# databio/IGD

Hardware: AMD Instinct MI355X
Metric: query-intervals/sec (igd search -q, hits-only) on roadmap-scale synthetic .igd (higher is better)
Workload: dtype int32; 1 GPU; BASELINE config 2: roadmap-scale synthetic IGD, 1900 files x 26316 intervals (53143736 tile records, 188505 tiles of 16384 bp, hg38 contigs) replicated per GPU + 1000000 position-sorted queries per step (seed 7), hits-only, queries and DB resident in HBM; queries_per_gpu=1000000, parallelism=query-sharded x1, grouping=sorted, query_layout=contig numbers + starts + ends (12 B/query; igd_hip_search_dev), collective=none

## Files before the change

### igd_amd/csrc/engine/host_search.hpp

```cpp

static int ensure_workspace(igd_hip_db *db, int64_t nq, int pairBytes)
{
    int rc;
    if (nq > db->wsQueries) {
        HIPCHK(hipDeviceSynchronize());
        if (db->d_fix) (void)hipFree(db->d_fix);
        if (db->d_qw) (void)hipFree(db->d_qw);
        if (db->d_later) (void)hipFree(db->d_later);
        if (db->d_laterHdr) (void)hipFree(db->d_laterHdr);
        db->d_fix = nullptr; db->d_qw = nullptr; db->d_later = nullptr; db->d_laterHdr = nullptr;
        db->wsQueries = 0;
        if ((rc = dalloc(&db->d_fix, (size_t)nq * 2, nullptr)) != IGD_HIP_OK) return rc;
        if ((rc = dalloc(&db->d_qw, (size_t)nq + 64, nullptr)) != IGD_HIP_OK) return rc;
        if ((rc = dalloc(&db->d_later, (size_t)nq + 4096 + 64, nullptr)) != IGD_HIP_OK) return rc;
        if ((rc = dalloc(&db->d_laterHdr, 2 * ((size_t)nq / 256 + 2), nullptr)) != IGD_HIP_OK) return rc;
        db->wsQueries = nq;
    }
    if (pairBytes == 0 || (nq <= db->wsBucket && pairBytes <= db->pairBytes)) return IGD_HIP_OK;
    HIPCHK(hipDeviceSynchronize());
    const int64_t cap = nq > db->wsBucket ? nq : db->wsBucket;
    const int pb = pairBytes > db->pairBytes ? pairBytes : db->pairBytes;
    {
        void *ws[] = { db->d_pairs, db->d_long, db->d_spTable, db->d_spT, db->d_spSub };
        for (void *q : ws) if (q) (void)hipFree(q);
        db->d_pairs = nullptr; db->d_long = nullptr; db->d_spTable = nullptr; db->d_spT = nullptr; db->d_spSub = nullptr;
    }
    db->wsBucket = 0;
    if ((rc = dalloc((char **)&db->d_pairs, (size_t)cap * IGD_SHORT_TILES * (size_t)pb, nullptr)) != IGD_HIP_OK) return rc;
    if ((rc = dalloc(&db->d_long, (size_t)cap, nullptr)) != IGD_HIP_OK) return rc;
    {
        int sh = SP_MINSHIFT;
        while (sh < 13 && ((db->nT + (1 << sh) - 1) >> sh) > SP_MAXC) sh++;
        db->spShift = (((db->nT + (1 << sh) - 1) >> sh) <= SP_MAXC && sh <= 12) ? sh : -1;
        db->spCoarse = db->spShift >= 0 ? (db->nT + (1 << sh) - 1) >> sh : 0;
        if (db->spShift >= 0) {
            const size_t nWG = (size_t)((cap + SP_Q - 1) / SP_Q);
            if ((rc = dalloc(&db->d_spTable, nWG * (size_t)db->spCoarse, nullptr)) != IGD_HIP_OK) return rc;
            if ((rc = dalloc(&db->d_spT, nWG * SP_CAP, nullptr)) != IGD_HIP_OK) return rc;
            const size_t subN = (((size_t)db->spCoarse * SPF_S) << db->spShift) + 2 * (size_t)db->spCoarse + 16;
            if ((rc = dalloc(&db->d_spSub, subN, nullptr)) != IGD_HIP_OK) return rc;
            HIPCHK(hipMemset(db->d_spSub, 0, subN * 4));
        }
    }
    db->wsBucket = cap;
    db->pairBytes = pb;
    return IGD_HIP_OK;
}

static int launch_bucket(igd_hip_db *db, const int32_t *d_ichr, const int32_t *d_qs, const int32_t *d_qe,
                         int nq, int rule, int gate, int packed, hipStream_t st, u64 *zeroHits = nullptr,
                         u64 *zeroTotal = nullptr)
{
    const int nT = db->nT;
    const int qb = (nq + 255) / 256;
    const int qbz = zeroHits ? ((nq > db->nFiles ? nq : db->nFiles) + 255) / 256 : qb;
    k_count_pairs<<<qbz, 256, 0, st>>>(db->v, d_ichr, d_qs, d_qe, nq, rule, packed, db->d_pairCnt, db->d_long, db->d_ctl,
                                      gate, db->epoch, zeroHits, zeroTotal);
    const int sb = (nT + IGD_SCAN_TILE - 1) / IGD_SCAN_TILE;
    k_scan_block_sums<<<sb, IGD_SCAN_BLOCK, 0, st>>>(db->d_pairCnt, nT, db->d_blockSums, db->d_ctl, gate);
    k_scan_apply<<<sb, IGD_SCAN_BLOCK, 0, st>>>(db->d_pairCnt, nT, db->d_blockSums, db->d_pairPos, db->d_pairN,
                                                db->d_ctl, gate);
    k_scatter_pairs<<<qb, 256, 0, st>>>(db->v, d_ichr, d_qs, d_qe, nq, rule, packed, db->d_pairPos, db->d_pairs,
                                                db->d_ctl, gate);
    HIPCHK(hipGetLastError());
    return IGD_HIP_OK;
}

static int launch_split(igd_hip_db *db, const int32_t *d_ichr, const int32_t *d_qs, const int32_t *d_qe,
                        int nq, int rule, int gate, int packed, hipStream_t st, u64 *zeroHits, u64 *zeroTotal)
{
    const int nWG = (nq + SP_Q - 1) / SP_Q;
    uint32_t *bases = db->d_spSub + (((size_t)db->spCoarse * SPF_S) << db->spShift);
    int32_t *blong = (int32_t *)(bases + db->spCoarse);
    const int bitsWords = (!db->splitNoBits && db->v.tileBits && db->nT <= 40 * 1024 * 8) ? (db->nT + 31) / 32 + 1 : 0;
    const int ctgStaged = (!db->splitNoBits && db->nCtg <= 1024) ? db->nCtg : 0;
    const int stageCap = (db->splitNoBits || db->splitNoRegion) ? 0 : SP_Q + SP_Q / 8;
    size_t ldsLocal = (size_t)bitsWords * 4 + (size_t)ctgStaged * 8;
    if (ldsLocal < (size_t)stageCap * 12 + 16) ldsLocal = (size_t)stageCap * 12 + 16;
    if (bitsWords && ctgStaged && db->v.vshift < 0 && db->v.shift >= 0 && db->spShift >= 2)
    k_split_local<true><<<nWG, SP_WG, ldsLocal, st>>>(db->v, d_ichr, d_qs, d_qe, nq, rule, packed, db->spShift, db->spCoarse, db->d_spTable,
                                         db->d_spT, db->d_long, db->d_ctl, gate, db->epoch, zeroHits, zeroTotal, blong, bitsWords, ctgStaged, stageCap);
    else
    k_split_local<false><<<nWG, SP_WG, ldsLocal, st>>>(db->v, d_ichr, d_qs, d_qe, nq, rule, packed, db->spShift, db->spCoarse, db->d_spTable,
                                         db->d_spT, db->d_long, db->d_ctl, gate, db->epoch, zeroHits, zeroTotal, blong, bitsWords, ctgStaged, stageCap);
    const size_t ldsCnt = (size_t)2 * 4 << db->spShift;
    int64_t cap = 2 * (((int64_t)nq + nq / 8) / db->spCoarse) + 256;
    if (cap < 1024) cap = 1024;
    if (cap > (int64_t)((65536 - 256 - ldsCnt) / 12)) cap = (int64_t)((65536 - 256 - ldsCnt) / 12);
    if (db->splitNoStage || cap < 256) cap = 0;
    k_split_fine_a<<<db->spCoarse * SPF_S, SPF_WG, ldsCnt + (size_t)cap * 12, st>>>(db->nT, db->spShift, db->spCoarse, nWG, db->d_spTable, db->d_spT,
        db->d_spSub, bases, blong, db->d_pairN, db->d_pairPos, (int2 *)db->d_pairs, db->d_ctl, gate, db->d_ctl, db->epoch, packed ? db->d_heavy : nullptr, (int)cap);
    k_split_fine_b<<<db->spCoarse * SPF_S < 512 ? db->spCoarse * SPF_S : 512, SPF_WG, (size_t)4 << db->spShift, st>>>(db->nT, db->spShift, db->spCoarse, nWG, db->d_spTable, db->d_spT,
        db->d_spSub, bases, blong, db->d_pairN, db->d_pairPos, (int2 *)db->d_pairs, db->d_ctl, gate, db->d_ctl, db->epoch, packed ? db->d_heavy : nullptr);
    HIPCHK(hipGetLastError());
    return IGD_HIP_OK;
}

static SortK make_sortk(igd_hip_db *db, const ScanArgs &a)
{
    SortArgs sa;
    sa.firstQ = a.firstQ; sa.spill = db->d_spill; sa.qw0 = db->d_qw; sa.later = db->d_later; sa.q_qs = a.q_qs; sa.ctl = a.ctl;
    sa.laterHdr = (const int2 *)db->d_laterHdr; sa.lbShift = db->lbShift; sa.lpos = db->d_lpos;
    sa.nq = a.nq; sa.v = a.v; sa.epoch = a.epoch; sa.mode = a.mode; sa.out = a.out; sa.rule = a.rule;
    sa.sbCap = db->sbCap; sa.wldsBytes = IGD_WLDS_BYTES + 2 * db->sbCap;
    sa.ctlw = db->d_ctl; sa.heavyS = db->d_heavy + IGD_HEAVY_MAX; sa.farList = db->d_far; sa.tailHistOff = -1; sa.noList = 0;
    SortK K;
    K.db = db->v; K.a = sa; K.hitsOut = (u64 *)a.hitsOut; K.totalOut = a.total;
    return K;
}

template <typename F, typename KA>
static void launch_sorted(igd_hip_db *db, F kernel, int grid, int block, size_t lds, hipStream_t st, const KA &K)
{
    if (db->evStart) {
        KA k = K;
        void *args[] = {&k};
        (void)hipExtLaunchKernel((const void *)kernel, dim3(grid), dim3(block), args, lds, st, db->evStart, db->evStop, 0);
        db->evStart = db->evStop = nullptr;
    } else kernel<<<grid, block, lds, st>>>(K);
}

template <bool USE_V, bool LDS_HITS, bool PACKED>
static void launch_scan(igd_hip_db *db, const ScanArgs &a, hipStream_t st, int win = -1)
{
    const int fileLo = win > 0 ? win * db->winN : 0;
    const int fileN = win >= 0 ? (db->nFiles - fileLo < db->winN ? db->nFiles - fileLo : db->winN) : db->nFiles;
    const size_t lds = LDS_HITS ? db->ldsBytes : 0;
    if (a.mode != 2 && PACKED) {
        const bool big = db->bigImage || db->nRec + IGD_CHUNK >= (1ll << 30);
        const size_t ldsS = (size_t)db->ldsSorted;
        SortK K = make_sortk(db, a);
        if (win >= 0) { K.db.nFiles = fileN; K.db.fileLo = fileLo; K.hitsOut += fileLo; K.a.noList = win > 0 ? 1 : 0; }
        const int forceRank = db->forceRank;
        bool lean = forceRank >= 0 ? forceRank == 0 : ((int64_t)a.nq < 28ll * db->nT && (int64_t)a.nq >= (int64_t)db->nT);
        const int64_t wavesLean = (int64_t)db->grid * (IGD_WG_LEAN / IGD_WAVE);
        if (((int64_t)db->nUnits + wavesLean - 1) / wavesLean * (IGD_WG_LEAN / IGD_WAVE) * (IGD_LEAN_FIRST + IGD_WAVE) * IGD_CHUNK >= (1ll << 32)) lean = false;
        const int few = (LDS_HITS && !big) ? (win >= 0 ? 3 : db->nFiles == 1 ? 1 : db->nFiles <= 8 ? 2 : 0) : 0;
        if (big) launch_sorted(db, igd_scan_sorted<USE_V, LDS_HITS, LDS_HITS, true, true>, db->grid, IGD_WG_RANK, ldsS, st, K);
        else if (lean) {
            const size_t l = LDS_HITS ? ldsS : 0;
            if (few == 1) launch_sorted(db, igd_scan_sorted<USE_V, LDS_HITS, LDS_HITS, false, false, LDS_HITS ? 1 : 0>, db->grid, IGD_WG_LEAN, l, st, K);
            else if (few == 2) launch_sorted(db, igd_scan_sorted<USE_V, LDS_HITS, LDS_HITS, false, false, LDS_HITS ? 2 : 0>, db->grid, IGD_WG_LEAN, l, st, K);
            else if (few == 3) launch_sorted(db, igd_scan_sorted<USE_V, LDS_HITS, LDS_HITS, false, false, LDS_HITS ? 3 : 0>, db->grid, IGD_WG_LEAN, l, st, K);
            else launch_sorted(db, igd_scan_sorted<USE_V, LDS_HITS, LDS_HITS, false, false>, db->grid, IGD_WG_LEAN, l, st, K);
        } else {
            if (few == 1) launch_sorted(db, igd_scan_sorted<USE_V, LDS_HITS, LDS_HITS, false, true, LDS_HITS ? 1 : 0>, db->grid, IGD_WG_RANK, ldsS, st, K);
            else if (few == 2) launch_sorted(db, igd_scan_sorted<USE_V, LDS_HITS, LDS_HITS, false, true, LDS_HITS ? 2 : 0>, db->grid, IGD_WG_RANK, ldsS, st, K);
            else if (few == 3) launch_sorted(db, igd_scan_sorted<USE_V, LDS_HITS, LDS_HITS, false, true, LDS_HITS ? 3 : 0>, db->grid, IGD_WG_RANK, ldsS, st, K);
            else launch_sorted(db, igd_scan_sorted<USE_V, LDS_HITS, LDS_HITS, false, true>, db->grid, IGD_WG_RANK, ldsS, st, K);
        }
    } else
    if (a.mode != 2) {
        if (win >= 0) { DbView v = db->v; v.nFiles = fileN; v.fileLo = fileLo; igd_scan_tiles<true, USE_V, LDS_HITS, PACKED, LDS_HITS><<<db->grid, IGD_WG, lds, st>>>(v, a); }
        else igd_scan_tiles<true, USE_V, LDS_HITS, PACKED><<<db->grid, IGD_WG, lds, st>>>(db->v, a);
    }
    if (a.mode != 1) {
        if (win >= 0) { DbView v = db->v; v.nFiles = fileN; v.fileLo = fileLo; igd_scan_tiles<false, USE_V, LDS_HITS, PACKED, LDS_HITS><<<db->grid, IGD_WG, lds, st>>>(v, a); }
        else igd_scan_tiles<false, USE_V, LDS_HITS, PACKED><<<db->grid, IGD_WG, lds, st>>>(db->v, a);
    }
}
template <bool LDS_HITS>
static void launch_scan_any(igd_hip_db *db, const ScanArgs &a, bool useV, bool packed, hipStream_t st, int win = -1)
{
    if (packed) {
        if (useV) launch_scan<true, LDS_HITS, true>(db, a, st, win); else launch_scan<false, LDS_HITS, true>(db, a, st, win);
    } else {
        if (useV) launch_scan<true, LDS_HITS, false>(db, a, st, win); else launch_scan<false, LDS_HITS, false>(db, a, st, win);
    }
}

__global__ void k_expand_runs(const int32_t *__restrict__ runs, int nCtg, int32_t *__restrict__ ichr, int nq)
{
    const int i = blockIdx.x * blockDim.x + threadIdx.x;
    if (i >= nq) return;
    int lo = 0, hi = nCtg;
    while (hi - lo > 1) { const int mid = (lo + hi) >> 1; if (runs[mid] <= i) lo = mid; else hi = mid; }
    ichr[i] = lo;
}

static int search_dev_impl(igd_hip_db *db, const int32_t *d_ichr, const int32_t *d_runs, const int32_t *d_qs,
                           const int32_t *d_qe, int64_t nq, int32_t v, int rule, int flags,
                           int64_t *d_hits, int64_t *d_total, void *stream);

extern "C" int igd_hip_search_dev(igd_hip_db *db, const int32_t *d_ichr, const int32_t *d_qs,
                                  const int32_t *d_qe, int64_t nq, int32_t v, int rule, int flags,
                                  int64_t *d_hits, int64_t *d_total, void *stream)
{
    return search_dev_impl(db, d_ichr, nullptr, d_qs, d_qe, nq, v, rule, flags, d_hits, d_total, stream);
}

extern "C" int igd_hip_search_runs_dev(igd_hip_db *db, const int32_t *d_run_start, const int32_t *d_qs,
                                       const int32_t *d_qe, int64_t nq, int32_t v, int rule, int flags,
                                       int64_t *d_hits, int64_t *d_total, void *stream)
{
    if (!d_run_start || (flags & IGD_HIP_FLAG_BUCKET)) {
        snprintf(g_err, sizeof g_err, "igd_hip_search_runs_dev: bad argument");
        return IGD_HIP_ERR_ARG;
    }
    return search_dev_impl(db, nullptr, d_run_start, d_qs, d_qe, nq, v, rule, flags | IGD_HIP_FLAG_SORTED, d_hits, d_total, stream);
}

static int search_dev_impl(igd_hip_db *db, const int32_t *d_ichr, const int32_t *d_runs, const int32_t *d_qs,
                           const int32_t *d_qe, int64_t nq, int32_t v, int rule, int flags,
                           int64_t *d_hits, int64_t *d_total, void *stream)
{
    if (!db || !d_hits || nq < 0 || nq > IGD_MAX_BATCH || (rule != IGD_HIP_RULE_NEST && rule != IGD_HIP_RULE_FLAT) ||
        ((flags & IGD_HIP_FLAG_SORTED) && (flags & IGD_HIP_FLAG_BUCKET))) {
        snprintf(g_err, sizeof g_err, "igd_hip_search_dev: bad argument");
        return IGD_HIP_ERR_ARG;
    }
    if (db->nFiles == 0) return IGD_HIP_OK;
    if (db->inner) {
        db->inner->vnest = rule == IGD_HIP_RULE_NEST ? 1 : 0;
        return search_dev_impl(db->inner, d_ichr, d_runs, d_qs, d_qe, nq, v, IGD_HIP_RULE_FLAT, flags, d_hits, d_total,
                               stream ? stream : (void *)db->stream);
    }
    HIPCHK(hipSetDevice(db->device));
    hipStream_t st = stream ? (hipStream_t)stream : db->stream;
    if (nq == 0 || db->nT == 0) {
        if (flags & IGD_HIP_FLAG_ZERO_FIRST) {
            HIPCHK(hipMemsetAsync(d_hits, 0, (size_t)db->nFiles * 8, st));
            if (d_total) HIPCHK(hipMemsetAsync(d_total, 0, 8, st));
        }
        return IGD_HIP_OK;
    }
    int rc = ensure_workspace(db, nq, (flags & IGD_HIP_FLAG_SORTED) ? 0 : 8);
    if (rc != IGD_HIP_OK) return rc;
    const bool useV = (v != IGD_HIP_NO_VALUE_FILTER && db->gType == 1);
    const int mode = (flags & IGD_HIP_FLAG_SORTED) ? 1 : (flags & IGD_HIP_FLAG_BUCKET) ? 2 : 0;
    const int krule = rule | ((db->v.vshift >= 0 && db->vnest) ? 0x100 : 0);
    const bool packed = db->packed && !(flags & IGD_HIP_FLAG_EXACT) && (!useV || db->packedV);
    if (db->epoch >= 0x3fffffff || db->covStale) {
        HIPCHK(hipMemsetAsync(db->d_spill, 0, ((size_t)db->nT + 2) * 4, st));
        HIPCHK(hipMemsetAsync(db->d_cov, 0, 4 * IGD_COV_LEN(db->nT) * 4, st));
        HIPCHK(hipMemsetAsync(db->d_ctl + CTL_COV, 0, 4 * 4, st));
        if (db->d_spSub && db->spShift >= 0)
            HIPCHK(hipMemsetAsync(db->d_spSub + (((size_t)db->spCoarse * SPF_S) << db->spShift) + db->spCoarse, 0, (size_t)db->spCoarse * 4, st));
        if (!db->covStale) db->epoch = 0;
        db->covStale = false;
    }
    db->epoch++;
    struct StaleGuard { igd_hip_db *d; bool done; ~StaleGuard() { if (!done) d->covStale = true; } } guard{db, false};
    int slot = -1;
    if (db->evOn && db->evUsed < db->evMax && (db->evSeen++ % (db->evEvery > 0 ? db->evEvery : 1)) == 0) slot = db->evUsed++;
    const bool pipeEv = slot >= 0 && slot < IGD_PIPE_EVENTS;
    if (pipeEv) HIPCHK(hipEventRecord(db->ev[4 * slot + 0], st));
    u64 *zh = (flags & IGD_HIP_FLAG_ZERO_FIRST) ? (u64 *)d_hits : nullptr;
    u64 *zt = (flags & IGD_HIP_FLAG_ZERO_FIRST) ? (u64 *)d_total : nullptr;
    const bool direct = mode == 1 && packed && db->ldsHits && db->nWin == 1 && db->v.tileD != nullptr && db->v.vshift < 0 && db->v.shift >= 0 && db->nCtg <= QB_CTG &&
                        (db->forceDirect > 0 || (db->forceDirect < 0 && (flags & IGD_HIP_FLAG_SHORT) && nq >= 28ll * db->nT));
    db->lastDirect = direct ? 1 : 0;
    if (mode != 2) {
        bool vec = ((((uintptr_t)d_ichr) | ((uintptr_t)d_qs) | ((uintptr_t)d_qe)) & 15) == 0;
        const bool fast = packed && db->v.shift >= 0 && db->nCtg <= QB_CTG;
        if (nq < 65536) vec = false;
        bool runsK = d_runs != nullptr && vec && fast;
        if (d_runs && !runsK) {
            if (nq > db->runCap) {
                HIPCHK(hipStreamSynchronize(st));
                if (db->d_runIchr) (void)hipFree(db->d_runIchr);
                db->d_runIchr = nullptr; db->runCap = 0;
                if ((rc = dalloc(&db->d_runIchr, (size_t)nq, nullptr)) != IGD_HIP_OK) return rc;
                db->runCap = nq;
            }
            k_expand_runs<<<(int)((nq + 255) / 256), 256, 0, st>>>(d_runs, db->nCtg, db->d_runIchr, (int)nq);
            d_ichr = db->d_runIchr;
            vec = vec && (((uintptr_t)d_ichr) & 15) == 0;
        }
        const int fillBlocks = (int)((db->nT >> 10) < 256 ? (db->nT >> 10) + 1 : 256);
        const bool wide = vec && nq >= ((int64_t)1 << 22);
#define QB_GRID(PER_) ((int)((nq + (PER_) - 1) / (PER_)) > fillBlocks ? (int)((nq + (PER_) - 1) / (PER_)) : fillBlocks)
#define QB_LAUNCH(VEC_, FAST_, WGT_)                                                                                                  \
    if (direct && FAST_ && runsK && VEC_ == 4)                                         \
        k_query_bounds<4, true, WGT_, true, true><<<QB_GRID(WGT_ * 4), WGT_, 0, st>>>(db->v, d_runs, d_qs, d_qe, (int)nq, krule,      \
        1, db->d_firstQ, db->d_lpos, db->d_fix, db->d_ctl, db->epoch, zh, zt, db->d_qw, db->d_later, db->d_spill,                      \
        (int2 *)db->d_laterHdr, 1);                                                                                                  \
    else if (direct && FAST_)                                                                                                        \
        k_query_bounds<VEC_, true, WGT_, false, true><<<QB_GRID(WGT_ * VEC_), WGT_, 0, st>>>(db->v, d_ichr, d_qs, d_qe, (int)nq, krule, \
        1, db->d_firstQ, db->d_lpos, db->d_fix, db->d_ctl, db->epoch, zh, zt, db->d_qw, db->d_later, db->d_spill,                      \
        (int2 *)db->d_laterHdr, 1);                                                                                                  \
    else if (runsK && VEC_ == 4 && FAST_)                                                                                             \
        k_query_bounds<4, true, WGT_, true><<<QB_GRID(WGT_ * 4), WGT_, 0, st>>>(db->v, d_runs, d_qs, d_qe, (int)nq, krule,            \
        packed ? 1 : 0, db->d_firstQ, db->d_lpos, db->d_fix, db->d_ctl, db->epoch, zh, zt, db->d_qw, db->d_later, db->d_spill,         \
        (int2 *)db->d_laterHdr, mode == 1 ? 1 : 0);                                                                                  \
    else                                                                                                                             \
    k_query_bounds<VEC_, FAST_, WGT_><<<QB_GRID(WGT_ * VEC_), WGT_, 0, st>>>(db->v, d_ichr, d_qs, d_qe, (int)nq, krule,               \
        packed ? 1 : 0, db->d_firstQ, db->d_lpos, db->d_fix, db->d_ctl, db->epoch, zh, zt, db->d_qw, db->d_later, db->d_spill,         \
        (int2 *)db->d_laterHdr, mode == 1 ? 1 : 0)
        if (wide && !direct) { if (fast) QB_LAUNCH(4, true, 1024); else QB_LAUNCH(4, false, 1024); }
        else if (vec) { if (fast) QB_LAUNCH(4, true, 256); else QB_LAUNCH(4, false, 256); }
        else { if (fast) QB_LAUNCH(1, true, 256); else QB_LAUNCH(1, false, 256); }
#undef QB_LAUNCH
#undef QB_GRID
        db->lbShift = wide ? 12 : vec ? 10 : 8;
    }
    if (mode != 1) {
        if (db->spShift >= 0)
            rc = launch_split(db, d_ichr, d_qs, d_qe, (int)nq, krule, mode == 2 ? 0 : db->epoch, packed ? 1 : 0, st,
                              mode == 2 ? zh : nullptr, mode == 2 ? zt : nullptr);
        else
            rc = launch_bucket(db, d_ichr, d_qs, d_qe, (int)nq, krule, mode == 2 ? 0 : db->epoch, packed ? 1 : 0, st,
                                      mode == 2 ? zh : nullptr, mode == 2 ? zt : nullptr);
        if (rc != IGD_HIP_OK) return rc;
    }
    const bool extEv = slot >= 0 && mode == 1 && packed && db->ldsHits && db->nWin == 1;
    if (slot >= 0 && !extEv) HIPCHK(hipEventRecord(db->ev[4 * slot + 1], st));
    ScanArgs a;
    a.firstQ = db->d_firstQ; a.pairN = db->d_pairN; a.pairPos = db->d_pairPos; a.pairs = (const int2 *)db->d_pairs;
    a.walkList = nullptr; a.ctl = db->d_ctl; a.q_ichr = d_ichr; a.q_qs = d_qs; a.q_qe = d_qe; a.q_w = db->d_qw;
    a.total = (u64 *)d_total; a.hitsOut = (u64 *)d_hits;
    a.nq = (int)nq; a.v = v; a.rule = rule; a.epoch = db->epoch; a.mode = mode;
    a.packedWalk = packed ? (useV ? 2 : 1) : 0;
    const int valves = direct ? 8 : (mode != 1 && packed && db->spShift >= 0 ? 1 : 0) | (mode != 2 && packed ? 2 : 0) |
                       (db->bigImage || db->nRec + IGD_CHUNK >= (1ll << 30) ? 4 : 0);
    const size_t tailWave = direct ? (size_t)IGD_D_WLDS : (size_t)IGD_WLDS_BYTES;
    size_t tailLds = (valves & (2 | 8)) ? (size_t)(db->ldsHits ? IGD_TAIL_WG / IGD_WAVE : 4) * tailWave : 0;
    int tailHistOff = -1;
    if ((size_t)db->nFiles * 8 <= (size_t)48 * 1024) { tailHistOff = (int)tailLds; tailLds += (size_t)db->nFiles * 8; }
    if (db->ldsHits) {
        a.out = db->d_slab;
        const SortK K = make_sortk(db, a);
        for (int win = 0; win < db->nWin; win++) {
            const bool last = win == db->nWin - 1;
            const int fileLo = win * db->winN, fileN = db->nWin == 1 ? db->nFiles : (db->nFiles - fileLo < db->winN ? db->nFiles - fileLo : db->winN);
            if (extEv) { db->evStart = db->ev[4 * slot + 1]; db->evStop = db->ev[4 * slot + 2]; }
            if (direct) {
                DirK D;
                D.db = db->v;
                D.a.firstQ = db->d_firstQ; D.a.tileD = db->v.tileD; D.a.q_qs = d_qs; D.a.q_qe = d_qe; D.a.ctl = db->d_ctl; D.a.fix = db->d_fix;
                D.a.heavyS = db->d_heavy + IGD_HEAVY_MAX; D.a.farList = db->d_far; D.a.nq = (int)nq; D.a.v = v; D.a.epoch = db->epoch;
                D.a.rule = rule; D.a.promised = 1; D.a.sbCap = db->sbCap; D.a.wldsBytes = IGD_D_WLDS + 2 * db->sbCap;
                D.a.out = db->d_slab; D.a.hitsOut = (u64 *)d_hits; D.a.totalOut = (u64 *)d_total;
                if (useV) launch_sorted(db, igd_scan_direct<true>, db->grid, IGD_WG_DIR, (size_t)db->ldsDirect, st, D);
                else launch_sorted(db, igd_scan_direct<false>, db->grid, IGD_WG_DIR, (size_t)db->ldsDirect, st, D);
            } else
            launch_scan_any<true>(db, a, useV, packed, st, db->nWin > 1 ? win : -1);
            if (extEv && db->evStart) {
                db->evStart = db->evStop = nullptr;
                HIPCHK(hipEventRecord(db->ev[4 * slot + 1], st)); HIPCHK(hipEventRecord(db->ev[4 * slot + 2], st));
            }
            if (slot >= 0 && last && !extEv) HIPCHK(hipEventRecord(db->ev[4 * slot + 2], st));
            ScanArgs w = a;
            w.out = (u64 *)d_hits;
            SortK Kt = K;
            Kt.a.sbCap = 0; Kt.a.wldsBytes = (int)tailWave; Kt.a.tailHistOff = tailHistOff;
            const int gx = (fileN + IGD_TAIL_WG - 1) / IGD_TAIL_WG;
            dim3 rg(gx, (!last || IGD_REDUCE_GROUPS * gx >= IGD_TAIL_WGS) ? IGD_REDUCE_GROUPS : (IGD_TAIL_WGS + gx - 1) / gx);
            const int rows32 = (mode != 2 && packed) ? db->epoch : 0;
            if (useV)
                k_reduce_slabs<true><<<rg, IGD_TAIL_WG, last ? tailLds : 0, st>>>(Kt, db->d_slab, db->grid, fileN, (u64 *)d_hits + fileLo, (u64 *)d_total,
                                                               db->d_ctl, mode == 1 ? db->epoch : 0, w, db->d_fix, db->d_long, db->d_heavy, last ? valves : -1, rows32);
            else
                k_reduce_slabs<false><<<rg, IGD_TAIL_WG, last ? tailLds : 0, st>>>(Kt, db->d_slab, db->grid, fileN, (u64 *)d_hits + fileLo, (u64 *)d_total,
                                                                db->d_ctl, mode == 1 ? db->epoch : 0, w, db->d_fix, db->d_long, db->d_heavy, last ? valves : -1, rows32);
        }
    } else {
        a.out = (u64 *)d_hits;
        const SortK K = make_sortk(db, a);
        if (d_total) k_sum_hits<<<1, 256, 0, st>>>((const u64 *)d_hits, db->nFiles, (u64 *)d_total, -1);
        launch_scan_any<false>(db, a, useV, packed, st);
        if (slot >= 0) HIPCHK(hipEventRecord(db->ev[4 * slot + 2], st));
        {
            ScanArgs w = a;
            w.total = nullptr;
            SortK Kt = K;
            Kt.a.sbCap = 0; Kt.a.wldsBytes = IGD_WLDS_BYTES; Kt.a.tailHistOff = tailHistOff;
            if (useV) k_exact_walk<true><<<1024, 256, tailLds, st>>>(Kt, w, db->d_fix, db->d_long, db->d_heavy, valves);
            else k_exact_walk<false><<<1024, 256, tailLds, st>>>(Kt, w, db->d_fix, db->d_long, db->d_heavy, valves);
        }
        if (d_total) k_sum_hits<<<1, 256, 0, st>>>((const u64 *)d_hits, db->nFiles, (u64 *)d_total, +1);
    }
    if (pipeEv) HIPCHK(hipEventRecord(db->ev[4 * slot + 3], st));
    if (mode == 1) db->promised = db->epoch;
    db->lastMode = mode; db->lastPacked = packed ? 1 : 0;
    HIPCHK(hipGetLastError());
    guard.done = true;
    return IGD_HIP_OK;
}

extern "C" int igd_hip_sync(igd_hip_db *db, void *stream)
{
    if (!db) return IGD_HIP_ERR_ARG;
    if (db->inner) return igd_hip_sync(db->inner, stream ? stream : (void *)db->stream);
    HIPCHK(hipSetDevice(db->device));
    HIPCHK(hipStreamSynchronize(stream ? (hipStream_t)stream : db->stream));
    HIPCHK(hipGetLastError());
    if (db->promised) {
        int32_t ctl[4] = {0, 0, 0, 0};
        HIPCHK(hipMemcpy(ctl, db->d_ctl, sizeof ctl, hipMemcpyDeviceToHost));
        const bool broken = ctl[CTL_BROKEN] != 0;
        db->promised = 0;
        if (broken) {
            const int32_t zero = 0;
            HIPCHK(hipMemcpy(db->d_ctl + CTL_BROKEN, &zero, 4, hipMemcpyHostToDevice));
            snprintf(g_err, sizeof g_err, "igd_hip: queries passed with IGD_HIP_FLAG_SORTED were not ordered by "
                     "(contig, start); such a batch added nothing to hits");
            return IGD_HIP_ERR_UNSORTED;
        }
    }
    return IGD_HIP_OK;
}

extern "C" int igd_hip_sync_spin(igd_hip_db *db, void *stream)
{
    if (!db) return IGD_HIP_ERR_ARG;
    HIPCHK(hipSetDevice(db->device));
    hipStream_t st = stream ? (hipStream_t)stream : db->stream;
    for (;;) {
        const hipError_t e = hipStreamQuery(st);
        if (e == hipSuccess) break;
        if (e != hipErrorNotReady) { set_err("hipStreamQuery", e, __FILE__, __LINE__); return IGD_HIP_ERR_DEVICE; }
    }
    return igd_hip_sync(db, stream);
}

static int ensure_qstage(igd_hip_db *db, int64_t nq)
{
    if (nq <= db->qcap) return IGD_HIP_OK;
    HIPCHK(hipDeviceSynchronize());
    if (db->d_qc) (void)hipFree(db->d_qc);
    if (db->d_qs) (void)hipFree(db->d_qs);
    if (db->d_qe) (void)hipFree(db->d_qe);
    db->d_qc = db->d_qs = db->d_qe = nullptr;
    db->qcap = 0;
    int rc;
    if ((rc = dalloc(&db->d_qc, (size_t)nq, nullptr)) != IGD_HIP_OK) return rc;
    if ((rc = dalloc(&db->d_qs, (size_t)nq, nullptr)) != IGD_HIP_OK) return rc;
    if ((rc = dalloc(&db->d_qe, (size_t)nq, nullptr)) != IGD_HIP_OK) return rc;
    db->qcap = nq;
    return IGD_HIP_OK;
}

extern "C" int igd_hip_search(igd_hip_db *db, const int32_t *ichr, const int32_t *qs, const int32_t *qe,
                              int64_t nq, int32_t v, int rule, int64_t *hits, int64_t *total)
{
    return igd_hip_search_ex(db, ichr, qs, qe, nq, v, rule, 0, hits, total);
}

static int search_slab_resident(igd_hip_db *db, const int32_t *ichr, const int32_t *qs, const int32_t *qe,
// ... 53 lines not shown
```

### igd_amd/csrc/engine/scan_sorted.hpp

```cpp
#ifndef IGD_DENSE_MIN
#define IGD_DENSE_MIN 32
#endif

#define IGD_WLDS_S 512
#define IGD_WLDS_H 328
#define IGD_WLDS_BYTES (IGD_WLDS_S * 2 + IGD_WLDS_H * 4)

struct SortArgs {
    const int32_t *firstQ;
    const int32_t *spill;
    const int32_t *qw0, *later;
    const int32_t *lpos;
    const int2 *laterHdr;
    int lbShift;
    const int32_t *q_qs;
    const int32_t *ctl;
    int nq, v, epoch, mode, rule;
    int sbCap, wldsBytes;
    int32_t *ctlw, *heavyS;
    int32_t *farList;
    int noList;
    int tailHistOff;
    u64 *out;
};
// ... 314 lines not shown
            int qs2 = (int)((unsigned)w >> 16);
            const bool good = (unsigned)w != IGD_NEVER && qe2 >= qs2;
            const int pos = (IGD_EXP & 128) ? (qe2 & 255) : lds_lower_bound(sl, qe2);
            if (good) atomicAdd(&hist[pos], 1u);
            const unsigned long long gm = __ballot(good);
            nFirst += __popcll(gm);
            if (gm != ~0ull) batchFix(w, qs2, idx, ~gm);
            if (inLds) sb[idx] = (unsigned short)qs2;
        };
        if (nE <= IGD_WAVE) batchA(R.q, R.lw, 0, nl != 0);
        else {
            const __amdgpu_buffer_rsrc_t rsq = __builtin_amdgcn_make_buffer_rsrc((void *)a.qw0, 0, (f0 + c0) * 4, 0x00020000);
            const int vo4 = lane * 4;
            int wn = ~(int)__builtin_amdgcn_raw_buffer_load_b32(rsq, vo4, (f0 + IGD_WAVE - nl) * 4, 0);
            batchA(R.q, R.lw, 0, nl != 0);
            int p = IGD_WAVE;
            for (; p + IGD_WAVE <= nE; p += IGD_WAVE) {
                const int w = wn;
                wn = ~(int)__builtin_amdgcn_raw_buffer_load_b32(rsq, vo4, (f0 + p + IGD_WAVE - nl) * 4, 0);
                batchIn(w, p);
            }
            if (p < nE) batchA(wn, 0, p, false);
        }
        if (far)
            far_later<true>(a, __builtin_amdgcn_readlane(L.la, kk), ln, f0, lane, [&](int e) {
                bool covers;
                const int key = later_end(db.nbp, e, g2, deadk, true, covers);
#if IGD_EXP & 512
                nLater += __popcll(__ballot(covers));
                return;
#endif
                const int pos = (IGD_EXP & 128) ? (key & 255) : lds_lower_bound(sl, key);
                if (covers) atomicAdd(&hist[pos], 1u);
                nLater += __popcll(__ballot(covers));
            });
        __builtin_amdgcn_fence(__ATOMIC_ACQ_REL, "wavefront");
        __builtin_amdgcn_wave_barrier();
        {
            const int levels = 32 - __builtin_clz((unsigned)c0), top = 1 << levels;
            int pos[IGD_SLOTS];
            bool inLdsDone = false;
#pragma unroll
            for (int r = 0; r < IGD_SLOTS; r++) pos[r] = 0;
            if (IGD_EXP & 64) {
            } else
            if (inLds) {
                for (int k = c0 + lane; k < top - 1; k += IGD_WAVE) sb[k] = 65535;
                __builtin_amdgcn_fence(__ATOMIC_ACQ_REL, "wavefront");
                __builtin_amdgcn_wave_barrier();
                typedef __attribute__((address_space(3))) const unsigned short *lds_u16;
                const unsigned sb0 = (unsigned)(size_t)(lds_u16)sb;
                unsigned Q[IGD_SLOTS], E[IGD_SLOTS];
                const unsigned q0 = sb0 + (unsigned)top - 2u;
#pragma unroll
                for (int r = 0; r < IGD_SLOTS; r++) { Q[r] = q0; E[r] = R.a[r] >> 16; }
                int vq[IGD_SLOTS];
                for (int S = top >> 1; S > 1; S >>= 1) {
                    const int up = S, dn = -S;
#pragma unroll
                    for (int r = 0; r < IGD_SLOTS; r++) vq[r] = (int)*(lds_u16)(size_t)Q[r];
#pragma unroll
                    for (int r = 0; r < IGD_SLOTS; r++) Q[r] += (unsigned)(vq[r] <= (int)E[r] ? up : dn);
                }
#pragma unroll
                for (int r = 0; r < IGD_SLOTS; r++) vq[r] = (int)*(lds_u16)(size_t)Q[r];
                const unsigned zero = sb0 + 2u * (unsigned)c0;
#pragma unroll
                for (int r = 0; r < IGD_SLOTS; r++) cnt[r] += ((int)(Q[r] - zero) >> 1) + (vq[r] <= (int)E[r] ? 1 : 0);
                inLdsDone = true;
            } else {
                const int32_t *q_qs = KARG(a.q_qs);
                const int T = IGD_TILE_START;
                for (int step = top >> 1; step > 0; step >>= 1) {
                    int vq[IGD_SLOTS];
#pragma unroll
                    for (int r = 0; r < IGD_SLOTS; r++) {
                        const int at = pos[r] + step - 1;
                        vq[r] = at < c0 ? q_qs[f0 + at] : INT_MAX;
                    }
#pragma unroll
                    for (int r = 0; r < IGD_SLOTS; r++) pos[r] += vq[r] <= (int)(R.a[r] >> 16) + T - 1 ? step : 0;
                }
            }
            if (!inLdsDone) {
#pragma unroll
                for (int r = 0; r < IGD_SLOTS; r++) cnt[r] -= c0 - pos[r];
            }
        }
        int carry = 0;
#pragma unroll
        for (int r = 0; r < IGD_SLOTS; r++) {
            const int h = (int)hist[r * IGD_WAVE + lane];
            hist[r * IGD_WAVE + lane] = 0u;
            const int inc = (IGD_EXP & 256) ? h : wave_inclusive_sum(h);
            const bool prefix = (R.a[r] & 0xFFFFu) == 0xFFFFu;
            cnt[r] += nFirst + (prefix ? 0 : nLater) - (carry + inc);
            carry += __builtin_amdgcn_readlane(inc, 63);
            if (R.a[r] == 0u || !keep[r]) cnt[r] = 0;
        }
        if (lane == 0) hist[IGD_SLOTS * IGD_WAVE] = 0u;
#undef IGD_TILE_START
    }
    if (FEW == 3) {
#pragma unroll
        for (int r = 0; r < IGD_SLOTS; r++) {
            const unsigned x = (unsigned)R.x[r] - (unsigned)db.fileLo;
            const bool in = x < (unsigned)db.nFiles;
            cnt[r] = in ? cnt[r] : 0;
            R.x[r] = in ? (int)x : 0;
        }
    }
    bool direct = !CNT32;
    if (CNT32 && RANK) {
        long long cand = nE;
        if (IGD_LN_FAR(ln)) {
            const int bA = __builtin_amdgcn_readlane(L.la, kk) >> a.lbShift, bB = f0 >> a.lbShift;
            cand += IGD_LN_A(ln) + IGD_LN_B(ln) + (bB - bA > 1 ? (long long)(bB - bA - 1) << a.lbShift : 0);
        }
        const long long bound = cand * un;
        direct = bound > (long long)(budget - *spent);
        if (!direct) *spent += (unsigned)bound;
    }
    if (!direct && FEW == 1) {
        int s = 0;
#pragma unroll
        for (int r = 0; r < IGD_SLOTS; r++) s += cnt[r];
        s = wave_inclusive_sum(s);
        if (lane == IGD_WAVE - 1 && s) atomicAdd((unsigned int *)hits, (unsigned)s);
    } else
    if (!direct) {
        constexpr bool few = FEW != 0;
#pragma unroll
        for (int r = 0; r < IGD_SLOTS; r++) {
#if IGD_EXP & 1
            asm volatile("" ::"v"(cnt[r]), "v"(R.x[r]));
            continue;
#endif
            if (!RANK && !few && !USE_V) {
                unsigned off;
                asm("v_mad_u32_u16 %0, %1, 4, 0" : "=v"(off) : "v"(R.x[r]));
                atomicAdd((unsigned int *)((char *)hits + off), (unsigned)cnt[r]);
            } else
            if ((!RANK && !few) || cnt[r]) atomicAdd((unsigned int *)hits + R.x[r], (unsigned)cnt[r]);
        }
    } else
    if (LDSH && lhits) {
#pragma unroll
        for (int r = 0; r < IGD_SLOTS; r++) {
            const int c = cnt[r];
            if (c) (void)__hip_atomic_fetch_add(lhits + R.x[r], (u64)(unsigned)c, __ATOMIC_RELAXED, __HIP_MEMORY_SCOPE_WORKGROUP);
        }
    } else {
        u64 *gh = CNT32 ? KARG(hitsOut) : hits;
        if (CNT32) found = KARG(totalOut);
#pragma unroll
        for (int r = 0; r < IGD_SLOTS; r++) {
            const int c = cnt[r];
            if (c) atomicAdd((u64 *)((char *)gh + ((size_t)R.x[r] << 3)), (u64)(unsigned)c);
        }
    }
    if (found) {
        int t = 0;
#pragma unroll
        for (int r = 0; r < IGD_SLOTS; r++) t += cnt[r];
        for (int o = 32; o > 0; o >>= 1) t += __shfl_down(t, o);
        if (lane == 0 && t) atomicAdd(found, (u64)(unsigned)t);
    }
}

template <bool USE_V, int NS>
__device__ __forceinline__ void s_compute_small(const DbView &db, const SortArgs &a, const SRegs &L, int kk, int lane, Raw2 &R, u64 *hits)
{
    const int c0 = R.c0, ln = R.ln, f0 = R.f0;
    int cnt[NS];
#pragma unroll
    for (int r = 0; r < NS; r++) cnt[r] = 0;
    if (USE_V) {
#pragma unroll
        for (int r = 0; r < NS; r++) {
            if ((R.x[r] >> 16) < a.v) R.a[r] = 0u;
            R.x[r] &= 0xFFFF;
        }
    }
    const int nl = IGD_LN_A(ln) + IGD_LN_B(ln);
    int g2 = 0, deadk = 0, nLater = 0;
    if (ln) {
        g2 = IGD_LN_G2(ln);
        deadk = a.rule == IGD_HIP_RULE_NEST ? (__builtin_amdgcn_readlane(L.jf, kk) & 14) : 0;
    }
    const int nE = nl + c0;
    uint32_t W[NS];
#pragma unroll
    for (int r = 0; r < NS; r++) W[r] = (uint32_t)__builtin_amdgcn_readlane(L.w[r], kk);
    int w = R.q;
    if (nl) {
        bool covers;
        const int lw = later_word(db.nbp, R.lw, g2, deadk, lane < nl, covers);
        nLater = __popcll(__ballot(covers));
        w = lane < nl ? lw : w;
    }
    auto match = [&](int P0) {
#pragma unroll
        for (int r = 0; r < NS; r++) match_slot_asm<false>(cnt[r], W[r], P0, R.a[r], 0ull);
    };
    if (nE > IGD_WAVE) {
        int wn = (IGD_WAVE + lane < nE) ? ~a.qw0[f0 + IGD_WAVE + lane - nl] : (int)IGD_NEVER;
        match(w);
        for (int p = IGD_WAVE; p < nE; p += IGD_WAVE) {
            w = wn;
            wn = (p + IGD_WAVE + lane < nE) ? ~a.qw0[f0 + p + IGD_WAVE + lane - nl] : (int)IGD_NEVER;
            match(w);
        }
    } else if (nE > 0) match(w);
    if (nLater != 0) {
#pragma unroll
        for (int r = 0; r < NS; r++) cnt[r] -= (R.a[r] & 0xFFFFu) == 0xFFFFu ? nLater : 0;
    }
#pragma unroll
    for (int r = 0; r < NS; r++) {
        if (!USE_V) {
            unsigned off;
            asm("v_mad_u32_u16 %0, %1, 4, 0" : "=v"(off) : "v"(R.x[r]));
            atomicAdd((unsigned int *)((char *)hits + off), (unsigned)cnt[r]);
        } else atomicAdd((unsigned int *)hits + R.x[r], (unsigned)cnt[r]);
    }
}

template <bool USE_V, bool CNT32, bool LDS_HITS, int FEW>
__device__ __forceinline__ void s_compute_lean(const DbView &db, const SortArgs &a, const SRegs &L, int kk, int lane, Raw2 &R,
                                               u64 *hits, unsigned short *sl, unsigned int *hist, unsigned short *sb, bool rankOK,
                                               unsigned *spent, unsigned budget)
{
#if IGD_EXP == 0 && !IGD_EXP_NOMATCH
    if (CNT32 && LDS_HITS && FEW == 0) {
        const int un = R.n;
        if (un == 0) return;
        if (un <= IGD_WAVE) { s_compute_small<USE_V, 1>(db, a, L, kk, lane, R, hits); return; }
        if (un <= 3 * IGD_WAVE) { s_compute_small<USE_V, 3>(db, a, L, kk, lane, R, hits); return; }
    }
#endif
    s_compute<USE_V, CNT32, false, LDS_HITS, FEW>(db, a, L, kk, lane, R, hits, sl, hist, sb, rankOK, nullptr, spent, budget);
}

#ifndef IGD_WG_RANK
#define IGD_WG_RANK 768
#define IGD_WPE_RANK 6
#endif
#define IGD_ROUND 62
#ifndef IGD_WG_LEAN
#define IGD_WG_LEAN IGD_WG
#define IGD_WPE_LEAN IGD_WPE
#endif
template <bool USE_V, bool LDS_HITS, bool CNT32, bool BIG, bool RANK, int FEW = 0>
__global__ __launch_bounds__(RANK ? IGD_WG_RANK : IGD_WG_LEAN)
__attribute__((amdgpu_waves_per_eu(RANK ? IGD_WPE_RANK : IGD_WPE_LEAN, RANK ? IGD_WPE_RANK : IGD_WPE_LEAN))) void igd_scan_sorted(SortK K)
{
    constexpr int WGT = RANK ? IGD_WG_RANK : IGD_WG_LEAN;
    const DbView &db = K.db;
    const SortArgs &a = K.a;
    bool rankOK;
    {
        const int32_t *ctl = KARG(a.ctl);
        if (__builtin_amdgcn_readfirstlane(ctl[CTL_UNSORTED]) == a.epoch) return;
        rankOK = __builtin_amdgcn_readfirstlane(ctl[CTL_NOTSTART]) != a.epoch;
    }
    extern __shared__ __attribute__((aligned(16))) unsigned char smem[];
    const int lane = threadIdx.x & 63;
    const int wid = __builtin_amdgcn_readfirstlane((int)(threadIdx.x >> 6));
    u64 *hits;
    unsigned short *sl;
    {
        const int nFiles = KARG(db.nFiles);
        const size_t hitBytes = LDS_HITS ? (((size_t)nFiles * (CNT32 ? 4 : 8) + 15) & ~(size_t)15) : 0;
        hits = LDS_HITS ? (u64 *)smem : KARG(a.out);
        sl = (unsigned short *)(smem + hitBytes + (size_t)wid * (size_t)KARG(a.wldsBytes));
        if (LDS_HITS) {
            if (CNT32) for (int f = threadIdx.x; f < nFiles; f += WGT) ((unsigned int *)hits)[f] = 0u;
            else for (int f = threadIdx.x; f < nFiles; f += WGT) hits[f] = 0;
        }
    }
    unsigned int *hist = (unsigned int *)(sl + IGD_WLDS_S);
    unsigned short *sb = (unsigned short *)(hist + IGD_WLDS_H);
    if (RANK) {
        for (int k = lane; k < IGD_WLDS_S; k += IGD_WAVE) sl[k] = 65535;
        for (int k = lane; k < IGD_WLDS_H; k += IGD_WAVE) hist[k] = 0u;
    }
    if (LDS_HITS) __syncthreads();
    const int wavesPerWG = WGT / IGD_WAVE;
    const int gwave = (int)blockIdx.x * wavesPerWG + wid;
    const int nwaves = gridDim.x * wavesPerWG;
    Raw2 A, B;
    unsigned spent = 0u;
    const unsigned budget = 0xFFFFFFFFu / (unsigned)(WGT / IGD_WAVE);
    const int myUnits = (db.nUnits - gwave + nwaves - 1) / nwaves;
    const int quarter = (myUnits + 3) >> 2;
    int prioAt = quarter, prioLevel = 3, done = 0;
    __builtin_amdgcn_s_setprio(3);

    for (int ub = gwave; ub < db.nUnits; ub += nwaves * IGD_ROUND) {
        SRegs L;
        L.offLo = L.offHi = L.n = L.jf = L.f0 = L.c0 = L.la = L.ln = 0;
#pragma unroll
        for (int r = 0; r < IGD_SLOTS; r++) L.w[r] = 0;
        {
            const long long mi = (long long)ub + (long long)lane * nwaves;
            if (lane < IGD_ROUND && mi < db.nUnits) {
                const Unit *units = KARG(db.units);
                const int32_t *firstQ = KARG(a.firstQ), *spill = KARG(a.spill);
                const UnitRegs u = load_unit_regs(units + mi);
                L.offLo = u.offLo; L.offHi = u.offHi; L.jf = u.jf;
                L.n = u.n;
#pragma unroll
                for (int r = 0; r < IGD_SLOTS; r++) L.w[r] = u.w[r];
                if (u.n > 0) {
                    const int lj = u.jf >> 4;
                    const int lb = lj < IGD_SHORT_TILES - 1 ? lj : IGD_SHORT_TILES - 1;
                    L.f0 = firstQ[u.tile];
                    L.c0 = firstQ[u.tile + 1] - L.f0;
                    if (spill[u.tile] == a.epoch) later_range<true>(a, u.tile, lb, firstQ[u.tile - lb], L.f0, L.la, L.ln);
                    const bool heavy = L.c0 > (RANK ? IGD_HEAVY_FIRST : IGD_LEAN_FIRST);
                    if (heavy) {
                        if ((u.jf & 1) && !a.noList) KARG(a.heavyS)[atomicAdd(&KARG(a.ctlw)[CTL_NHEAVYS + (a.epoch & 1)], 1)] = u.tile;
                        L.c0 = 0;
                    }
                    if (IGD_LN_FAR(L.ln) && (!RANK || (!BIG && (L.f0 >> a.lbShift) - (L.la >> a.lbShift) >= IGD_FAR_WIDE))) {
                        if (!a.noList) KARG(a.farList)[atomicAdd(&KARG(a.ctlw)[CTL_NFAR + (a.epoch & 1)], 1)] = (int)mi | (heavy ? (int)0x80000000 : 0);
                        L.c0 = 0; L.ln = 0;
                    }
                    if ((L.c0 | L.ln) == 0) L.n = 0;
                    if (!BIG) {
                        const int nlL = IGD_LN_FAR(L.ln) ? 0 : IGD_LN_A(L.ln) + IGD_LN_B(L.ln);
                        const int b0L = L.c0 < IGD_WAVE - nlL ? L.c0 : IGD_WAVE - nlL;
                        L.offHi = (L.f0 + b0L) * 4;
                    }
                }
            }
        }
        int cntU = (int)(((long long)db.nUnits - ub + nwaves - 1) / nwaves);
        if (cntU > IGD_ROUND) cntU = IGD_ROUND;
#define IGD_UNIT(kk_, R_) do { if (RANK) s_compute<USE_V, CNT32, RANK, LDS_HITS, FEW>(db, a, L, kk_, lane, R_, hits, sl, hist, sb, rankOK, nullptr, &spent, budget); \
                               else s_compute_lean<USE_V, CNT32, LDS_HITS, FEW>(db, a, L, kk_, lane, R_, hits, sl, hist, sb, rankOK, &spent, budget); } while (0)
        const unsigned long long mVis = __ballot((L.c0 | L.ln) != 0 && L.n > 0);
        if (RANK || __popcll(mVis) * 4 < cntU * 3) {
            unsigned long long m = mVis;
            const int visited = __popcll(m);
            int qd = (visited + 3) >> 2, at = qd, level = 3, nd = 0;
            __builtin_amdgcn_s_setprio(3);
            int ka = -1, kb = -1;
            if (m) { ka = __builtin_ctzll(m); m &= m - 1; }
            if (m) { kb = __builtin_ctzll(m); m &= m - 1; }
            s_issue<USE_V, BIG>(db, a, L, ka < 0 ? 0 : ka, ka >= 0, lane, A);
            while (ka >= 0) {
                s_issue<USE_V, BIG>(db, a, L, kb < 0 ? 0 : kb, kb >= 0, lane, B);
                s_compute<USE_V, CNT32, RANK, LDS_HITS, FEW>(db, a, L, ka, lane, A, hits, sl, hist, sb, rankOK, nullptr, &spent, budget);
                ka = -1;
                if (m) { ka = __builtin_ctzll(m); m &= m - 1; }
                s_issue<USE_V, BIG>(db, a, L, ka < 0 ? 0 : ka, ka >= 0, lane, A);
                if (kb >= 0) s_compute<USE_V, CNT32, RANK, LDS_HITS, FEW>(db, a, L, kb, lane, B, hits, sl, hist, sb, rankOK, nullptr, &spent, budget);
                kb = -1;
                if (m) { kb = __builtin_ctzll(m); m &= m - 1; }
                nd += 2;
                if (nd >= at) {
                    at += qd;
                    level--;
                    if (level == 2) __builtin_amdgcn_s_setprio(2);
                    else if (level == 1) __builtin_amdgcn_s_setprio(1);
                    else __builtin_amdgcn_s_setprio(0);
                }
            }
            continue;
        }
        s_issue<USE_V, BIG, !RANK>(db, a, L, 0, true, lane, A);
        for (int kk = 0; kk < cntU; kk += 2) {
            s_issue<USE_V, BIG, !RANK>(db, a, L, kk + 1, kk + 1 < cntU, lane, B);
            IGD_UNIT(kk, A);
            s_issue<USE_V, BIG, !RANK>(db, a, L, kk + 2, kk + 2 < cntU, lane, A);
            if (kk + 1 < cntU) IGD_UNIT(kk + 1, B);
            done += 2;
            if (done >= prioAt) {
                prioAt += quarter;
                prioLevel--;
                if (prioLevel == 2) __builtin_amdgcn_s_setprio(2);
                else if (prioLevel == 1) __builtin_amdgcn_s_setprio(1);
                else __builtin_amdgcn_s_setprio(0);
            }
        }
    }
    if (LDS_HITS) {
        __syncthreads();
        const int nFiles = KARG(db.nFiles);
        u64 *row = KARG(a.out) + (size_t)blockIdx.x * nFiles;
        if (CNT32) {
            unsigned int *row32 = (unsigned int *)KARG(a.out) + (size_t)blockIdx.x * nFiles;
            for (int f = threadIdx.x; f < nFiles; f += WGT) row32[f] = ((unsigned int *)hits)[f];
        } else for (int f = threadIdx.x; f < nFiles; f += WGT) row[f] = hits[f];
    }
}

#undef IGD_UNIT

template <bool USE_V, bool BIG>
__device__ __forceinline__ void heavy_sorted_body(const SortK &K, u64 *__restrict__ d_hits, u64 *__restrict__ d_total,
                                                  unsigned char *wsm, int gwave, int nwaves, int lane, int ctlv, igd_lds_u64 *lhits = nullptr)
{
    const DbView &db = K.db;
    const SortArgs &a = K.a;
    if (__builtin_amdgcn_readlane(ctlv, CTL_UNSORTED) == a.epoch) return;
    int nH = __builtin_amdgcn_readlane(ctlv, CTL_NHEAVYS + (a.epoch & 1));
    if (nH == 0) return;
    if (nH > IGD_HEAVYS_MAX) nH = IGD_HEAVYS_MAX;
    unsigned short *sl = (unsigned short *)wsm;
    unsigned int *hist = (unsigned int *)(sl + IGD_WLDS_S);
    unsigned short *sb = (unsigned short *)(hist + IGD_WLDS_H);
    for (int k = lane; k < IGD_WLDS_S; k += IGD_WAVE) sl[k] = 65535;
    for (int k = lane; k < IGD_WLDS_H; k += IGD_WAVE) hist[k] = 0u;
    const bool rankOK = __builtin_amdgcn_readlane(ctlv, CTL_NOTSTART) != a.epoch;
    int lf0 = 0, lc0 = 0, lu0 = 0, lnu = 0;
    deal_items(nH, gwave, nwaves, lane,
        [&](int h) {
            lf0 = lc0 = lu0 = lnu = 0;
            if (h < 0) return 0;
            const int tl = a.heavyS[h];
            lf0 = a.firstQ[tl]; lc0 = a.firstQ[tl + 1] - lf0;
            lu0 = db.tileUnit0[tl]; lnu = db.tileUnit0[tl + 1] - lu0;
            return lnu * ((lc0 + IGD_HEAVY_SLICE - 1) / IGD_HEAVY_SLICE);
        },
        [&](int hh, int it) {
            const int f0 = __builtin_amdgcn_readlane(lf0, hh), c0 = __builtin_amdgcn_readlane(lc0, hh);
            const int u0 = __builtin_amdgcn_readlane(lu0, hh), nu = __builtin_amdgcn_readlane(lnu, hh);
            const int u = u0 + it % nu, sc = it / nu;
            const UnitRegs ur = load_unit_regs(db.units + u);
            SRegs L;
            L.offLo = ur.offLo; L.offHi = ur.offHi; L.n = ur.n; L.jf = ur.jf;
#pragma unroll
            for (int r = 0; r < IGD_SLOTS; r++) L.w[r] = ur.w[r];
            L.f0 = f0 + sc * IGD_HEAVY_SLICE;
            L.c0 = c0 - sc * IGD_HEAVY_SLICE < IGD_HEAVY_SLICE ? c0 - sc * IGD_HEAVY_SLICE : IGD_HEAVY_SLICE;
            L.la = 0; L.ln = 0;
            Raw2 A;
            s_issue<USE_V, BIG>(db, a, L, 0, true, lane, A);
            s_compute<USE_V, false, true, true>(db, a, L, 0, lane, A, d_hits, sl, hist, sb, rankOK, d_total, nullptr, 0u, lhits);
        });
}

template <bool USE_V, bool BIG>
__device__ __forceinline__ void far_units_body(const SortK &K, u64 *__restrict__ d_hits, u64 *__restrict__ d_total,
                                               unsigned char *wsm, int gwave, int nwaves, int lane, int ctlv, igd_lds_u64 *lhits = nullptr)
{
    const DbView &db = K.db;
    const SortArgs &a = K.a;
    if (__builtin_amdgcn_readlane(ctlv, CTL_UNSORTED) == a.epoch) return;
    const int nF = __builtin_amdgcn_readlane(ctlv, CTL_NFAR + (a.epoch & 1));
    if (nF == 0) return;
    unsigned short *sl = (unsigned short *)wsm;
    unsigned int *hist = (unsigned int *)(sl + IGD_WLDS_S);
    unsigned short *sb = (unsigned short *)(hist + IGD_WLDS_H);
    for (int k = lane; k < IGD_WLDS_S; k += IGD_WAVE) sl[k] = 65535;
    for (int k = lane; k < IGD_WLDS_H; k += IGD_WAVE) hist[k] = 0u;
    const bool rankOK = __builtin_amdgcn_readlane(ctlv, CTL_NOTSTART) != a.epoch;
    if (nF > db.nUnits) return;
    int nS = nwaves / nF;
    nS = nS < 1 ? 1 : (nS > IGD_FAR_SLICES ? IGD_FAR_SLICES : nS);
    const int sh = a.lbShift;
    for (long long item = gwave; item < (long long)nF * nS; item += nwaves) {
        const int i = (int)(item / nS), sl_ = (int)(item % nS);
        const int ent = __builtin_amdgcn_readfirstlane(a.farList[i]);
        const UnitRegs ur = load_unit_regs(db.units + (ent & 0x7fffffff));
        SRegs L;
        L.offLo = ur.offLo; L.offHi = ur.offHi; L.n = ur.n; L.jf = ur.jf;
#pragma unroll
        for (int r = 0; r < IGD_SLOTS; r++) L.w[r] = ur.w[r];
        const int lj = ur.jf >> 4;
        const int lb = lj < IGD_SHORT_TILES - 1 ? lj : IGD_SHORT_TILES - 1;
        L.f0 = a.firstQ[ur.tile];
        L.c0 = (ent < 0 || sl_ > 0) ? 0 : a.firstQ[ur.tile + 1] - L.f0;
        later_range<false>(a, ur.tile, lb, a.firstQ[ur.tile - lb], L.f0, L.la, L.ln);
        if (nS > 1) {
            if (sl_ == 0) L.ln = 0;
            else if (L.ln != 0) {
                const int bA = L.la >> sh, bB = L.f0 >> sh;
                const int per = (bB - bA + nS - 1) / (nS - 1);
                const int b0 = bA + (sl_ - 1) * per;
                int b1 = b0 + per - 1;
                b1 = b1 > bB ? bB : b1;
                if (b0 > bB) continue;
                if (b0 != bA || b1 != bB) {
                    int nA = IGD_LN_A(L.ln), nB = IGD_LN_B(L.ln);
                    if (b0 != bA) { L.la = b0 << sh; nA = b0 == bB ? nB : a.laterHdr[b0].x; }
                    if (b1 != bB) { L.f0 = b1 << sh; nB = b1 == b0 ? 0 : a.laterHdr[b1].x; }
                    L.ln = (L.ln & ~0x3FFFFFF) | nA | (nB << 13);
                }
            }
        }
        if ((L.c0 | L.ln) == 0) continue;
        Raw2 A;
        s_issue<USE_V, BIG>(db, a, L, 0, true, lane, A);
        s_compute<USE_V, false, true, true>(db, a, L, 0, lane, A, d_hits, sl, hist, sb, rankOK, d_total, nullptr, 0u, lhits);
    }
}
```

Baseline: 12.31 billion query-intervals/s.

## Split leftover units into per-slot items dealt across waves in lean sorted scan

When the unit count does not divide evenly among waves, the lean non-big kernel now gives each wave its full share and breaks the remainder units into per-slot sub-items (one wave-width of records each), spread across all waves. The goal is to even out the tail imbalance where some waves process one extra whole unit. Sub-items whose queries spill past one wave fall back to the whole unit on slot 0, and heavy/far list insertion is restricted to slot 0 to avoid duplicates. The lean-eligibility overflow bound gains one extra round to cover the added items, so lean may be turned off in a few borderline cases.

```diff
diff --git a/igd_amd/csrc/engine/host_search.hpp b/igd_amd/csrc/engine/host_search.hpp
--- a/igd_amd/csrc/engine/host_search.hpp
+++ b/igd_amd/csrc/engine/host_search.hpp
@@ -134,7 +134,7 @@
         const int forceRank = db->forceRank;
         bool lean = forceRank >= 0 ? forceRank == 0 : ((int64_t)a.nq < 28ll * db->nT && (int64_t)a.nq >= (int64_t)db->nT);
         const int64_t wavesLean = (int64_t)db->grid * (IGD_WG_LEAN / IGD_WAVE);
-        if (((int64_t)db->nUnits + wavesLean - 1) / wavesLean * (IGD_WG_LEAN / IGD_WAVE) * (IGD_LEAN_FIRST + IGD_WAVE) * IGD_CHUNK >= (1ll << 32)) lean = false;
+        if ((((int64_t)db->nUnits + wavesLean - 1) / wavesLean + 1) * (IGD_WG_LEAN / IGD_WAVE) * (IGD_LEAN_FIRST + IGD_WAVE) * IGD_CHUNK >= (1ll << 32)) lean = false;
         const int few = (LDS_HITS && !big) ? (win >= 0 ? 3 : db->nFiles == 1 ? 1 : db->nFiles <= 8 ? 2 : 0) : 0;
         if (big) launch_sorted(db, igd_scan_sorted<USE_V, LDS_HITS, LDS_HITS, true, true>, db->grid, IGD_WG_RANK, ldsS, st, K);
         else if (lean) {
diff --git a/igd_amd/csrc/engine/scan_sorted.hpp b/igd_amd/csrc/engine/scan_sorted.hpp
--- a/igd_amd/csrc/engine/scan_sorted.hpp
+++ b/igd_amd/csrc/engine/scan_sorted.hpp
@@ -640,12 +640,43 @@
         L.offLo = L.offHi = L.n = L.jf = L.f0 = L.c0 = L.la = L.ln = 0;
 #pragma unroll
         for (int r = 0; r < IGD_SLOTS; r++) L.w[r] = 0;
+        constexpr bool SLOT_DEAL = !RANK && !BIG && CNT32 && LDS_HITS && FEW == 0;
+        int full = 0, rest = 0;
+        bool bySlot = false;
+        int nwv = nwaves, lanev = lane;
+        if (SLOT_DEAL) {
+            asm volatile("" : "+s"(nwv));
+            asm volatile("" : "+v"(lanev));
+            full = db.nUnits / nwv;
+            rest = db.nUnits - full * nwv;
+            bySlot = rest != 0 && full >= 4 && full + IGD_SLOTS <= IGD_ROUND;
+        }
+        int nItems = 0;
         {
-            const long long mi = (long long)ub + (long long)lane * nwaves;
-            if (lane < IGD_ROUND && mi < db.nUnits) {
+            long long mi = (long long)ub + (long long)lane * nwaves;
+            bool mine = lane < IGD_ROUND && mi < db.nUnits;
+            int slot = -1;
+            if (SLOT_DEAL && bySlot) {
+                const int item = (gwave >= rest ? gwave - rest : gwave - rest + nwv) + (lanev - full) * nwv;
+                mine = lanev < full;
+                if (lanev >= full && lanev < full + IGD_SLOTS && item < IGD_SLOTS * rest) {
+                    slot = (item >= rest ? 1 : 0) + (item >= 2 * rest ? 1 : 0) + (item >= 3 * rest ? 1 : 0) + (item >= 4 * rest ? 1 : 0);
+                    mi = (long long)full * nwv + (item - slot * rest);
+                    mine = true;
+                }
+                nItems = __popcll(__ballot(slot >= 0));
+            }
+            if (mine) {
                 const Unit *units = KARG(db.units);
                 const int32_t *firstQ = KARG(a.firstQ), *spill = KARG(a.spill);
-                const UnitRegs u = load_unit_regs(units + mi);
+                UnitRegs u = load_unit_regs(units + mi);
+                if (SLOT_DEAL && slot >= 0) {
+                    const int left = u.n - slot * IGD_WAVE;
+                    u.offLo += slot * IGD_WAVE;
+                    u.n = left < 0 ? 0 : (left < IGD_WAVE ? left : IGD_WAVE);
+#pragma unroll
+                    for (int r = 1; r < IGD_SLOTS; r++) { u.w[0] = slot == r ? u.w[r] : u.w[0]; u.w[r] = 0; }
+                }
                 L.offLo = u.offLo; L.offHi = u.offHi; L.jf = u.jf;
                 L.n = u.n;
 #pragma unroll
@@ -658,12 +689,21 @@
                     if (spill[u.tile] == a.epoch) later_range<true>(a, u.tile, lb, firstQ[u.tile - lb], L.f0, L.la, L.ln);
                     const bool heavy = L.c0 > (RANK ? IGD_HEAVY_FIRST : IGD_LEAN_FIRST);
                     if (heavy) {
-                        if ((u.jf & 1) && !a.noList) KARG(a.heavyS)[atomicAdd(&KARG(a.ctlw)[CTL_NHEAVYS + (a.epoch & 1)], 1)] = u.tile;
+                        if ((u.jf & 1) && !a.noList && slot <= 0) KARG(a.heavyS)[atomicAdd(&KARG(a.ctlw)[CTL_NHEAVYS + (a.epoch & 1)], 1)] = u.tile;
                         L.c0 = 0;
                     }
                     if (IGD_LN_FAR(L.ln) && (!RANK || (!BIG && (L.f0 >> a.lbShift) - (L.la >> a.lbShift) >= IGD_FAR_WIDE))) {
-                        if (!a.noList) KARG(a.farList)[atomicAdd(&KARG(a.ctlw)[CTL_NFAR + (a.epoch & 1)], 1)] = (int)mi | (heavy ? (int)0x80000000 : 0);
+                        if (!a.noList && slot <= 0) KARG(a.farList)[atomicAdd(&KARG(a.ctlw)[CTL_NFAR + (a.epoch & 1)], 1)] = (int)mi | (heavy ? (int)0x80000000 : 0);
                         L.c0 = 0; L.ln = 0;
+                    }
+                    if (SLOT_DEAL && slot >= 0 && (heavy || IGD_LN_A(L.ln) + IGD_LN_B(L.ln) + L.c0 > IGD_WAVE)) {
+                        if (slot != 0) { L.c0 = 0; L.ln = 0; }
+                        else {
+                            const UnitRegs o = load_unit_regs(units + mi);
+                            L.n = o.n;
+#pragma unroll
+                            for (int r = 0; r < IGD_SLOTS; r++) L.w[r] = o.w[r];
+                        }
                     }
                     if ((L.c0 | L.ln) == 0) L.n = 0;
                     if (!BIG) {
@@ -676,6 +716,7 @@
         }
         int cntU = (int)(((long long)db.nUnits - ub + nwaves - 1) / nwaves);
         if (cntU > IGD_ROUND) cntU = IGD_ROUND;
+        if (SLOT_DEAL && bySlot) cntU = full + nItems;
 #define IGD_UNIT(kk_, R_) do { if (RANK) s_compute<USE_V, CNT32, RANK, LDS_HITS, FEW>(db, a, L, kk_, lane, R_, hits, sl, hist, sb, rankOK, nullptr, &spent, budget); \
                                else s_compute_lean<USE_V, CNT32, LDS_HITS, FEW>(db, a, L, kk_, lane, R_, hits, sl, hist, sb, rankOK, &spent, budget); } while (0)
         const unsigned long long mVis = __ballot((L.c0 | L.ln) != 0 && L.n > 0);
```

Result: slower. 12.03 billion query-intervals/s (-2.2%).
